# bennyguo/instant-nsr-pl

Measured on NVIDIA H100. Metric: rays/sec fwd+bwd (NeRF-Synthetic lego shape), higher is better.
Workload: dtype f16

## Files before the change

instant-nsr-pl_b200/csrc/nerf_fused_bwd.cu:

```cuda
#include <stdlib.h>
#include "nerf_fused.cuh"
#include "wgmma.cuh"

namespace {

constexpr int kWarps = 4;
constexpr int kThreads = kWarps * 32;
constexpr int kRows = kWarps * 16;
constexpr int kCtasPerSm = 2;

constexpr int T_X0 = 0;
constexpr int T_H1 = T_X0 + kRows * NF_LD32;
constexpr int T_CI = T_H1 + kRows * NSR_LD64;
constexpr int T_G1 = T_CI + kRows * NF_LD32;
constexpr int T_G2 = T_G1 + kRows * NSR_LD64;
constexpr int T_DC3 = T_G2 + kRows * NSR_LD64;
constexpr int T_DG2 = T_DC3 + kRows * 24;
constexpr int T_DG1 = T_DG2 + kRows * NSR_LD64;
constexpr int T_DO = T_DG1 + kRows * NSR_LD64;
constexpr int T_DH1 = T_DO + kRows * 24;
constexpr int T_X0B = T_DH1 + kRows * NSR_LD64;
constexpr int T_TOTAL = T_X0B + kRows * NF_LD32;
constexpr int S_XYZ = 0, S_DS = S_XYZ + kRows * 6, S_DRGB = S_DS + kRows, S_ROWF = S_DRGB + kRows * 3;
constexpr size_t kSmemBytes = (size_t)(NF_W_TOTAL + T_TOTAL) * sizeof(__half) + 2 * S_ROWF * sizeof(float);

__device__ __forceinline__ void cp_async16(void* smem_dst, const void* gsrc) {
  asm volatile("cp.async.cg.shared.global [%0], [%1], 16;" ::"r"((uint32_t)__cvta_generic_to_shared(smem_dst)), "l"(gsrc) : "memory");
}
__device__ __forceinline__ void cp_async_commit() { asm volatile("cp.async.commit_group;" ::: "memory"); }
__device__ __forceinline__ void cp_async_wait_all() { asm volatile("cp.async.wait_group 0;" ::: "memory"); }

constexpr int kSlots = 40 / kWarps;

struct WgradTile {
  int dy_off, ldy, x_off, ldx, m0, n0;
  int net, base, in_dim;
};

__device__ __forceinline__ WgradTile wgrad_tile(int t) {
  WgradTile w;
  if (t < 8) {
    w = {T_DH1, NSR_LD64, T_X0, NF_LD32, (t / 2) * 16, (t % 2) * 16, 0, 0, 32};
  } else if (t < 12) {
    w = {T_DO, 24, T_H1, NSR_LD64, 0, (t - 8) * 16, 0, 64 * 32, 64};
  } else if (t < 20) {
    const int u = t - 12;
    w = {T_DG1, NSR_LD64, T_CI, NF_LD32, (u / 2) * 16, (u % 2) * 16, 1, 0, 32};
  } else if (t < 36) {
    const int u = t - 20;
    w = {T_DG2, NSR_LD64, T_G1, NSR_LD64, (u / 4) * 16, (u % 4) * 16, 1, 64 * 32, 64};
  } else {
    w = {T_DC3, 24, T_G2, NSR_LD64, 0, (t - 36) * 16, 1, 64 * 32 + 64 * 64, 64};
  }
  return w;
}

__device__ __forceinline__ void relu_mask_pack(const float (&acc)[1][8][4], const uint32_t (&post)[1][4][4], uint32_t (&out)[1][4][4]) {
#pragma unroll
  for (int k = 0; k < 4; ++k)
#pragma unroll
    for (int j = 0; j < 4; ++j) {
      const __half2 hv = *reinterpret_cast<const __half2*>(&post[0][k][j]);
      const int nt = 2 * k + (j >> 1), i0 = (j & 1) * 2;
      const float d0 = __low2float(hv) > 0.f ? acc[0][nt][i0] : 0.f;
      const float d1 = __high2float(hv) > 0.f ? acc[0][nt][i0 + 1] : 0.f;
      out[0][k][j] = nsr_pack_h2(d0, d1);
    }
}

template <bool PACKED>
__global__ void __launch_bounds__(kThreads, kCtasPerSm) nerf_bwd_kernel(const __grid_constant__ nsr_nerf_t P, const float* __restrict__ rays,
                                                               const int32_t* __restrict__ ray_indices, const float* __restrict__ t_starts,
                                                               const float* __restrict__ t_ends, const __half* __restrict__ enc_save,
                                                               const __half* __restrict__ dparams, const __half* __restrict__ cparams,
                                                               const float* __restrict__ d_sraw, const float* __restrict__ d_rgb,
                                                               float* __restrict__ grad_dparams, float* __restrict__ grad_cparams,
                                                               float loss_scale, const float* __restrict__ amax_ptr, int64_t n_cap, const int64_t* __restrict__ n_dev,
                                                               const int64_t* __restrict__ row_pos, const float* __restrict__ xyzdir) {
  const int64_t n = n_dev ? min(*n_dev, n_cap) : n_cap;
  extern __shared__ __align__(16) __half smem[];
  __half* T = smem + NF_W_TOTAL;
  float* rowf = reinterpret_cast<float*>(smem + NF_W_TOTAL + T_TOTAL);
  const int warp = threadIdx.x >> 5, lane = threadIdx.x & 31, g = lane >> 2, c = lane & 3;
  const int r0 = warp * 16;
  if (loss_scale <= 0.f) {
    const float amax = fmaxf(__ldg(amax_ptr), 1e-30f);
    loss_scale = exp2f(fminf(fmaxf(floorf(log2f(256.f / amax)), -24.f), 60.f));
  }
  const float inv_scale = 1.f / loss_scale;
  nf_stage_weights(smem, dparams, cparams, true);
  float* grad_table = grad_dparams + NF_DENSITY_PARAMS;

  float wacc[kSlots][2][4];
#pragma unroll
  for (int s = 0; s < kSlots; ++s)
#pragma unroll
    for (int j = 0; j < 2; ++j)
#pragma unroll
      for (int i = 0; i < 4; ++i) wacc[s][j][i] = 0.f;

  const int64_t n_tiles = (n + kRows - 1) / kRows;
  auto fetch_tile = [&](int64_t tile, int buf) {
    const int64_t row0 = tile * kRows;
    __half* xb = T + (buf ? T_X0B : T_X0);
    float* rf = rowf + buf * S_ROWF;
    for (int v = threadIdx.x; v < kRows * 4; v += kThreads)
      cp_async16(xb + (v >> 2) * NF_LD32 + (v & 3) * 8, enc_save + (row0 + (v >> 2)) * 32 + (v & 3) * 8);
    for (int v = threadIdx.x; v < kRows * 6 / 4; v += kThreads) cp_async16(rf + S_XYZ + v * 4, xyzdir + row0 * 6 + v * 4);
    if (threadIdx.x < kRows / 4) cp_async16(rf + S_DS + threadIdx.x * 4, d_sraw + row0 + threadIdx.x * 4);
    if (threadIdx.x >= 64 && threadIdx.x < 64 + kRows * 3 / 4)
      cp_async16(rf + S_DRGB + (threadIdx.x - 64) * 4, d_rgb + row0 * 3 + (threadIdx.x - 64) * 4);
    cp_async_commit();
  };
  int buf = 0;
  if (PACKED && (int64_t)blockIdx.x < n_tiles) fetch_tile(blockIdx.x, 0);
  for (int64_t tile = blockIdx.x; tile < n_tiles; tile += gridDim.x, buf ^= 1) {
    const int64_t row0 = tile * kRows;
    if (PACKED) cp_async_wait_all();
    __syncthreads();
    const __half* X0 = T + ((PACKED && buf) ? T_X0B : T_X0);
    const int x0_off = (PACKED && buf) ? T_X0B : T_X0;
    const float* rf = rowf + buf * S_ROWF;
    if (PACKED) {
      if (tile + gridDim.x < n_tiles) fetch_tile(tile + gridDim.x, buf ^ 1);
      if (row0 + kRows > n) {
        for (int v = threadIdx.x; v < kRows * 4; v += kThreads)
          if (row0 + (v >> 2) >= n) *reinterpret_cast<uint4*>(T + x0_off + (v >> 2) * NF_LD32 + (v & 3) * 8) = make_uint4(0, 0, 0, 0);
        float* rw = rowf + buf * S_ROWF;
        for (int v = threadIdx.x; v < S_ROWF; v += kThreads) {
          const int r = v < S_DS ? v / 6 : (v < S_DRGB ? v - S_DS : (v - S_DRGB) / 3);
          if (row0 + r >= n) rw[v] = 0.f;
        }
        __syncthreads();
      }
    }
    const int64_t ia = row0 + r0 + g, ib = ia + 8;
    const int64_t pa = (!PACKED && row_pos && ia < n) ? row_pos[ia] : ia, pb = (!PACKED && row_pos && ib < n) ? row_pos[ib] : ib;
    if (!PACKED) {
      for (int v = lane; v < 64; v += 32) {
        const int r = v >> 2, q = v & 3;
        const int64_t i = row0 + r0 + r;
        uint4 val = make_uint4(0, 0, 0, 0);
        if (i < n) val = __ldg(reinterpret_cast<const uint4*>(enc_save + (row_pos ? row_pos[i] : i) * 32) + q);
        *reinterpret_cast<uint4*>(T + T_X0 + (r0 + r) * NF_LD32 + q * 8) = val;
      }
    }
    if (lane < 16) {
      const int64_t i = row0 + r0 + lane;
      uint4 s0 = make_uint4(0, 0, 0, 0), s1 = s0;
      if (i < n) {
        float s[16];
        if (PACKED) {
          const float* rr = rf + S_XYZ + (r0 + lane) * 6;
          nsr_sh4(rr[3], rr[4], rr[5], s);
        } else {
          const float* rr = rays + (size_t)ray_indices[i] * 6;
          nsr_sh4(__ldg(rr + 3), __ldg(rr + 4), __ldg(rr + 5), s);
        }
        s0 = make_uint4(nsr_pack_h2(s[0], s[1]), nsr_pack_h2(s[2], s[3]), nsr_pack_h2(s[4], s[5]), nsr_pack_h2(s[6], s[7]));
        s1 = make_uint4(nsr_pack_h2(s[8], s[9]), nsr_pack_h2(s[10], s[11]), nsr_pack_h2(s[12], s[13]), nsr_pack_h2(s[14], s[15]));
      }
      uint4* sp = reinterpret_cast<uint4*>(T + T_CI + (r0 + lane) * NF_LD32 + 16);
      sp[0] = s0;
      sp[1] = s1;
    }
    __syncwarp();

    uint32_t a_h1[1][4][4], a_o[1][1][4], a_g1[1][4][4], a_g2[1][4][4];
    float acc[1][8][4], acc16[1][2][4];
    {
      uint32_t a_in[1][2][4];
      nsr_load_afrag<1, 2>(a_in, X0, NF_LD32, r0);
      nsr_zero_acc(acc);
      nsr_gemm_w<1, 2, 8>(acc, a_in, smem + NF_OFF_DW1, NF_LD32);
      nsr_acc_to_afrag<1, 8>(acc, a_h1, NSR_ACT_RELU);
      nsr_store_afrag<1, 4>(a_h1, T + T_H1, NSR_LD64, r0);
      nsr_zero_acc(acc16);
      nsr_gemm_w<1, 4, 2>(acc16, a_h1, smem + NF_OFF_DW2, NSR_LD64);
      nsr_acc_to_afrag<1, 2>(acc16, a_o, NSR_ACT_NONE);
      nsr_store_afrag<1, 1>(a_o, T + T_CI, NF_LD32, r0, 0);
    }
    {
      uint32_t a_c[1][2][4], a_sh[1][1][4];
      nsr_load_afrag<1, 1>(a_sh, T + T_CI + 16, NF_LD32, r0);
#pragma unroll
      for (int j = 0; j < 4; ++j) {
        a_c[0][0][j] = a_o[0][0][j];
        a_c[0][1][j] = a_sh[0][0][j];
      }
      nsr_zero_acc(acc);
      nsr_gemm_w<1, 2, 8>(acc, a_c, smem + NF_OFF_CW1, NF_LD32);
      nsr_acc_to_afrag<1, 8>(acc, a_g1, NSR_ACT_RELU);
      nsr_store_afrag<1, 4>(a_g1, T + T_G1, NSR_LD64, r0);
      nsr_zero_acc(acc);
      nsr_gemm_w<1, 4, 8>(acc, a_g1, smem + NF_OFF_CW2, NSR_LD64);
      nsr_acc_to_afrag<1, 8>(acc, a_g2, NSR_ACT_RELU);
      nsr_store_afrag<1, 4>(a_g2, T + T_G2, NSR_LD64, r0);
      nsr_zero_acc(acc16);
      nsr_gemm_w<1, 4, 2>(acc16, a_g2, smem + NF_OFF_CW3, NSR_LD64);
    }
    uint32_t a_dc3[1][1][4];
    {
      float dp[4] = {0.f, 0.f, 0.f, 0.f};
      if (c < 2) {
#pragma unroll
        for (int hh = 0; hh < 2; ++hh) {
          const int64_t i = hh ? ib : ia, pi = hh ? pb : pa;
          if (i < n) {
#pragma unroll
            for (int e = 0; e < 2; ++e) {
              const int col = c * 2 + e;
              if (col < 3) {
                const float raw = __half2float(__float2half_rn(acc16[0][0][hh * 2 + e]));
                const float s = 1.f / (1.f + expf(-raw));
                const float dr = PACKED ? rf[S_DRGB + (r0 + g + hh * 8) * 3 + col] : d_rgb[pi * 3 + col];
                dp[hh * 2 + e] = dr * s * (1.f - s) * loss_scale;
              }
            }
          }
        }
      }
      a_dc3[0][0][0] = nsr_pack_h2(dp[0], dp[1]);
      a_dc3[0][0][1] = nsr_pack_h2(dp[2], dp[3]);
      a_dc3[0][0][2] = 0u;
      a_dc3[0][0][3] = 0u;
      nsr_store_afrag<1, 1>(a_dc3, T + T_DC3, 24, r0);
    }
    uint32_t a_d[1][4][4];
    nsr_zero_acc(acc);
    nsr_gemm_wt<1, 1, 8>(acc, a_dc3, smem + NF_OFF_CW3, NSR_LD64);
    relu_mask_pack(acc, a_g2, a_d);
    nsr_store_afrag<1, 4>(a_d, T + T_DG2, NSR_LD64, r0);
    nsr_zero_acc(acc);
    nsr_gemm_wt<1, 4, 8>(acc, a_d, smem + NF_OFF_CW2, NSR_LD64);
    relu_mask_pack(acc, a_g1, a_d);
    nsr_store_afrag<1, 4>(a_d, T + T_DG1, NSR_LD64, r0);
    nsr_zero_acc(acc16);
    nsr_gemm_wt<1, 4, 2>(acc16, a_d, smem + NF_OFF_CW1, NF_LD32);
    if (c == 0) {
      if (ia < n) acc16[0][0][0] += (PACKED ? rf[S_DS + r0 + g] : d_sraw[pa]) * loss_scale;
      if (ib < n) acc16[0][0][2] += (PACKED ? rf[S_DS + r0 + g + 8] : d_sraw[pb]) * loss_scale;
    }
    uint32_t a_do[1][1][4];
    nsr_acc_to_afrag<1, 2>(acc16, a_do, NSR_ACT_NONE);
    nsr_store_afrag<1, 1>(a_do, T + T_DO, 24, r0);
    nsr_zero_acc(acc);
    nsr_gemm_wt<1, 1, 8>(acc, a_do, smem + NF_OFF_DW2, NSR_LD64);
    relu_mask_pack(acc, a_h1, a_d);
    nsr_store_afrag<1, 4>(a_d, T + T_DH1, NSR_LD64, r0);
    float accE[1][4][4];
    nsr_zero_acc(accE);
    nsr_gemm_wt<1, 4, 4>(accE, a_d, smem + NF_OFF_DW1, NF_LD32);

#pragma unroll
    for (int hh = 0; hh < 2; ++hh) {
      const int64_t i = hh ? ib : ia;
      const bool ok = i < n;
      float x = 0.f, y = 0.f, z = 0.f, dx, dy, dz;
      if (ok) {
        if (PACKED) {
          const float* rr = rf + S_XYZ + (r0 + g + hh * 8) * 6;
          x = rr[0];
          y = rr[1];
          z = rr[2];
        } else {
          nf_sample_position(P, rays, ray_indices[i], t_starts[i], t_ends[i], x, y, z, dx, dy, dz);
        }
      }
#pragma unroll
      for (int nt = 0; nt < 4; ++nt) {
        const float d0 = ok ? accE[0][nt][hh * 2] * inv_scale : 0.f, d1 = ok ? accE[0][nt][hh * 2 + 1] * inv_scale : 0.f;
        const LevelInfo li = nsr_level(P.grid, nt * 4 + c);
        uint32_t cx, cy, cz, idx[8];
        float fx, fy, fz;
        nsr_pos_fract(x, li.scale, cx, fx);
        nsr_pos_fract(y, li.scale, cy, fy);
        nsr_pos_fract(z, li.scale, cz, fz);
        if (nt < 2) {
          const uint32_t key = ok ? (cx + li.res * (cy + li.res * cz)) : (0xFFFFFFF0u + g);
          const uint32_t key_prev = __shfl_up_sync(0xffffffffu, key, 4);
          const bool head = (g == 0) || (key_prev != key);
          const int next_head = __shfl_down_sync(0xffffffffu, (int)head, 4);
          const bool tail = (g == 7) || next_head;
          float v[16];
#pragma unroll
          for (int cc = 0; cc < 8; ++cc) {
            const float w = nsr_corner_weight(cc, fx, fy, fz);
            v[2 * cc] = w * d0;
            v[2 * cc + 1] = w * d1;
          }
          bool flag = head;
#pragma unroll
          for (int o = 1; o < 8; o <<= 1) {
            const int f_up = __shfl_up_sync(0xffffffffu, (int)flag, 4 * o);
            const bool take = (g >= o) && !flag;
#pragma unroll
            for (int e = 0; e < 16; ++e) {
              const float u = __shfl_up_sync(0xffffffffu, v[e], 4 * o);
              if (take) v[e] += u;
            }
            if (take) flag = f_up;
          }
          if (ok && tail) {
            nsr_corner_indices(li, cx, cy, cz, idx);
#pragma unroll
            for (int cc = 0; cc < 8; ++cc)
              if (v[2 * cc] != 0.f || v[2 * cc + 1] != 0.f) nsr_red_add_f32x2(grad_table + 2 * (size_t)idx[cc], v[2 * cc], v[2 * cc + 1]);
          }
        } else if (ok && (d0 != 0.f || d1 != 0.f)) {
          nsr_corner_indices(li, cx, cy, cz, idx);
#pragma unroll
          for (int cc = 0; cc < 8; ++cc) {
            const float w = nsr_corner_weight(cc, fx, fy, fz);
            nsr_red_add_f32x2(grad_table + 2 * (size_t)idx[cc], w * d0, w * d1);
          }
        }
      }
    }
    __syncthreads();
#pragma unroll
    for (int s = 0; s < kSlots; ++s) {
      const WgradTile w = wgrad_tile(warp + s * kWarps);
      const int xo = (w.x_off == T_X0) ? x0_off : w.x_off;
      nsr_wgrad_tile(wacc[s][0], wacc[s][1], T + w.dy_off, w.ldy, w.m0, T + xo, w.ldx, w.n0, kRows);
    }
  }
#pragma unroll
  for (int s = 0; s < kSlots; ++s) {
    const WgradTile w = wgrad_tile(warp + s * kWarps);
    float* dst = (w.net == 0 ? grad_dparams : grad_cparams) + w.base;
#pragma unroll
    for (int j = 0; j < 2; ++j)
#pragma unroll
      for (int i = 0; i < 4; ++i) {
        const int o = w.m0 + g + ((i >> 1) << 3), ii = w.n0 + j * 8 + c * 2 + (i & 1);
        atomicAdd(dst + (size_t)o * w.in_dim + ii, wacc[s][j][i] * inv_scale);
      }
  }
}

constexpr int kNetThreads = 384;
constexpr int SL_X0 = 0;
constexpr int SL_CI = SL_X0 + kRows * 32 * 2;
constexpr int SL_H1 = SL_CI + kRows * 32 * 2;
constexpr int SL_G1 = SL_H1 + kRows * 64 * 2;
constexpr int SL_G2 = SL_G1 + kRows * 64 * 2;
constexpr int SL_DC3 = SL_G2 + kRows * 64 * 2;
constexpr int SL_DO = SL_DC3 + kRows * 16 * 2;
constexpr int SL_DG2 = SL_DO + kRows * 16 * 2;
constexpr int SL_DG1 = SL_DG2 + kRows * 64 * 2;
constexpr int SL_DH1 = SL_DG1 + kRows * 64 * 2;
constexpr int kSlotBytes = SL_DH1 + kRows * 64 * 2;
constexpr int kNetSlots = 3;
constexpr int N_SLOTS = NF_W_TOTAL * 2;
constexpr int N_STAGE = N_SLOTS + kNetSlots * kSlotBytes;
constexpr int kStageBytes = kRows * NF_LD32 * 2 + S_ROWF * 4;
constexpr int N_BARS = N_STAGE + 2 * kStageBytes;
constexpr size_t kNetSmemBytes = N_BARS + 2 * kNetSlots * 8;
static_assert(N_SLOTS % 128 == 0 && kSlotBytes % 128 == 0 && kStageBytes % 16 == 0 && N_BARS % 8 == 0, "alignment");
static_assert(kNetSmemBytes <= 227 * 1024, "shared memory");

template <int KT>
__device__ __forceinline__ void canon_load_afrag(uint32_t (&a)[1][KT][4], const uint8_t* tile, int K, int row0, int col0 = 0) {
  const int lane = threadIdx.x & 31, mi = lane >> 3, r = lane & 7;
#pragma unroll
  for (int k = 0; k < KT; ++k) nsr_ldmatrix_x4(a[0][k], tile + nsr_canon_off(row0 + (mi & 1) * 8 + r, col0 + k * 16 + (mi >> 1) * 8, K));
}
template <int KT>
__device__ __forceinline__ void canon_store_afrag(const uint32_t (&a)[1][KT][4], uint8_t* tile, int K, int row0, int col0 = 0) {
  const int lane = threadIdx.x & 31, g = lane >> 2, c = lane & 3;
#pragma unroll
  for (int k = 0; k < KT; ++k) {
    const int col = col0 + k * 16 + c * 2;
    *reinterpret_cast<uint32_t*>(tile + nsr_canon_off(row0 + g, col, K)) = a[0][k][0];
    *reinterpret_cast<uint32_t*>(tile + nsr_canon_off(row0 + g + 8, col, K)) = a[0][k][1];
    *reinterpret_cast<uint32_t*>(tile + nsr_canon_off(row0 + g, col + 8, K)) = a[0][k][2];
    *reinterpret_cast<uint32_t*>(tile + nsr_canon_off(row0 + g + 8, col + 8, K)) = a[0][k][3];
  }
}
__device__ __forceinline__ void group_bar(int grp) { asm volatile("bar.sync %0, 128;" ::"r"(1 + grp) : "memory"); }

template <int R>
__device__ __forceinline__ void net_flush(const float (&w)[R], float* dst, int stride_m, int stride_n, float inv_scale) {
  const int lane = threadIdx.x & 31, m0 = 16 * ((threadIdx.x >> 5) & 3) + (lane >> 2), c0 = 2 * (lane & 3);
#pragma unroll
  for (int r = 0; r < R; ++r) {
    const int j = r >> 2, h = (r >> 1) & 1, e = r & 1;
    atomicAdd(dst + (size_t)(m0 + 8 * h) * stride_m + (size_t)(8 * j + c0 + e) * stride_n, w[r] * inv_scale);
  }
}

__global__ void __launch_bounds__(kNetThreads, 1) nerf_bwd_net_kernel(const __half* __restrict__ enc_save, const __half* __restrict__ dparams,
                                                                      const __half* __restrict__ cparams, const float* __restrict__ d_sraw,
                                                                      const float* __restrict__ d_rgb, float* __restrict__ grad_dparams,
                                                                      float* __restrict__ grad_cparams, float loss_scale,
                                                                      const float* __restrict__ amax_ptr, int64_t n_cap,
                                                                      const int64_t* __restrict__ n_dev, const float* __restrict__ xyzdir,
                                                                      uint32_t* __restrict__ denc_out) {
  const int64_t n = n_dev ? min(*n_dev, n_cap) : n_cap;
  extern __shared__ __align__(128) uint8_t smem_net[];
  __half* W = reinterpret_cast<__half*>(smem_net);
  const int warp = threadIdx.x >> 5, lane = threadIdx.x & 31;
  if (loss_scale <= 0.f) {
    const float amax = fmaxf(__ldg(amax_ptr), 1e-30f);
    loss_scale = exp2f(fminf(fmaxf(floorf(log2f(256.f / amax)), -24.f), 60.f));
  }
  const float inv_scale = 1.f / loss_scale;
  const uint32_t sbase = nsr_smem_u32(smem_net);
  auto full_bar = [&](int s) { return sbase + N_BARS + 8u * (uint32_t)s; };
  auto empty_bar = [&](int s) { return sbase + N_BARS + 8u * (uint32_t)(kNetSlots + s); };
  if (threadIdx.x == 0) {
    for (int s = 0; s < kNetSlots; ++s) {
      mbar_init(full_bar(s), 128);
      mbar_init(empty_bar(s), 128);
    }
    asm volatile("fence.mbarrier_init.release.cluster;" ::: "memory");
  }
  nf_stage_weights(W, dparams, cparams, true);
  __syncthreads();
  const int64_t n_tiles = (n + kRows - 1) / kRows;
  const int64_t my_tiles = n_tiles > (int64_t)blockIdx.x ? (n_tiles - 1 - blockIdx.x) / gridDim.x + 1 : 0;

  if (warp < 8) {
    const int grp = warp >> 2, gtid = threadIdx.x & 127, g = lane >> 2, c = lane & 3;
    const int r0 = (warp & 3) * 16;
    __half* sx = reinterpret_cast<__half*>(smem_net + N_STAGE + grp * kStageBytes);
    float* rf = reinterpret_cast<float*>(smem_net + N_STAGE + grp * kStageBytes + kRows * NF_LD32 * 2);
    auto fetch_tile = [&](int64_t it) {
      const int64_t row0 = ((int64_t)blockIdx.x + it * gridDim.x) * kRows;
      for (int v = gtid; v < kRows * 4; v += 128) cp_async16(sx + (v >> 2) * NF_LD32 + (v & 3) * 8, enc_save + (row0 + (v >> 2)) * 32 + (v & 3) * 8);
      if (gtid < kRows * 6 / 4) cp_async16(rf + S_XYZ + gtid * 4, xyzdir + row0 * 6 + gtid * 4);
      if (gtid < kRows / 4) cp_async16(rf + S_DS + gtid * 4, d_sraw + row0 + gtid * 4);
      if (gtid >= 64 && gtid < 64 + kRows * 3 / 4) cp_async16(rf + S_DRGB + (gtid - 64) * 4, d_rgb + row0 * 3 + (gtid - 64) * 4);
      cp_async_commit();
    };
    if (grp < my_tiles) fetch_tile(grp);
    for (int64_t it = grp; it < my_tiles; it += 2) {
      const int s = (int)(it % kNetSlots);
      const int64_t row0 = ((int64_t)blockIdx.x + it * gridDim.x) * kRows;
      cp_async_wait_all();
      group_bar(grp);
      if (row0 + kRows > n) {
        for (int v = gtid; v < kRows * 4; v += 128)
          if (row0 + (v >> 2) >= n) *reinterpret_cast<uint4*>(sx + (v >> 2) * NF_LD32 + (v & 3) * 8) = make_uint4(0, 0, 0, 0);
        for (int v = gtid; v < S_ROWF; v += 128) {
          const int r = v < S_DS ? v / 6 : (v < S_DRGB ? v - S_DS : (v - S_DRGB) / 3);
          if (row0 + r >= n) rf[v] = 0.f;
        }
        group_bar(grp);
      }
      if (it >= kNetSlots) mbar_wait(empty_bar(s), (uint32_t)((it / kNetSlots - 1) & 1), nullptr, 0);
      uint8_t* slot = smem_net + N_SLOTS + s * kSlotBytes;
      const int64_t ia = row0 + r0 + g, ib = ia + 8;
      uint32_t a_in[1][2][4];
      nsr_load_afrag<1, 2>(a_in, sx, NF_LD32, r0);
      canon_store_afrag<2>(a_in, slot + SL_X0, 32, r0);
      if (lane < 16) {
        uint4 s0 = make_uint4(0, 0, 0, 0), s1 = s0;
        if (row0 + r0 + lane < n) {
          float sh[16];
          const float* rr = rf + S_XYZ + (r0 + lane) * 6;
          nsr_sh4(rr[3], rr[4], rr[5], sh);
          s0 = make_uint4(nsr_pack_h2(sh[0], sh[1]), nsr_pack_h2(sh[2], sh[3]), nsr_pack_h2(sh[4], sh[5]), nsr_pack_h2(sh[6], sh[7]));
          s1 = make_uint4(nsr_pack_h2(sh[8], sh[9]), nsr_pack_h2(sh[10], sh[11]), nsr_pack_h2(sh[12], sh[13]), nsr_pack_h2(sh[14], sh[15]));
        }
        *reinterpret_cast<uint4*>(slot + SL_CI + nsr_canon_off(r0 + lane, 16, 32)) = s0;
        *reinterpret_cast<uint4*>(slot + SL_CI + nsr_canon_off(r0 + lane, 24, 32)) = s1;
      }
      float drgb[2][2], dsr[2];
#pragma unroll
      for (int hh = 0; hh < 2; ++hh) {
#pragma unroll
        for (int e = 0; e < 2; ++e) drgb[hh][e] = (c * 2 + e < 3) ? rf[S_DRGB + (r0 + g + hh * 8) * 3 + c * 2 + e] : 0.f;
        dsr[hh] = rf[S_DS + r0 + g + hh * 8];
      }
      group_bar(grp);
      if (it + 2 < my_tiles) fetch_tile(it + 2);

      uint32_t a_h1[1][4][4], a_o[1][1][4], a_g1[1][4][4], a_g2[1][4][4];
      float acc[1][8][4], acc16[1][2][4];
      nsr_zero_acc(acc);
      nsr_gemm_w<1, 2, 8>(acc, a_in, W + NF_OFF_DW1, NF_LD32);
      nsr_acc_to_afrag<1, 8>(acc, a_h1, NSR_ACT_RELU);
      canon_store_afrag<4>(a_h1, slot + SL_H1, 64, r0);
      nsr_zero_acc(acc16);
      nsr_gemm_w<1, 4, 2>(acc16, a_h1, W + NF_OFF_DW2, NSR_LD64);
      nsr_acc_to_afrag<1, 2>(acc16, a_o, NSR_ACT_NONE);
      canon_store_afrag<1>(a_o, slot + SL_CI, 32, r0);
      __syncwarp();
      {
        uint32_t a_c[1][2][4], a_sh[1][1][4];
        canon_load_afrag<1>(a_sh, slot + SL_CI, 32, r0, 16);
#pragma unroll
        for (int j = 0; j < 4; ++j) {
          a_c[0][0][j] = a_o[0][0][j];
          a_c[0][1][j] = a_sh[0][0][j];
        }
        nsr_zero_acc(acc);
        nsr_gemm_w<1, 2, 8>(acc, a_c, W + NF_OFF_CW1, NF_LD32);
      }
      nsr_acc_to_afrag<1, 8>(acc, a_g1, NSR_ACT_RELU);
      canon_store_afrag<4>(a_g1, slot + SL_G1, 64, r0);
      nsr_zero_acc(acc);
      nsr_gemm_w<1, 4, 8>(acc, a_g1, W + NF_OFF_CW2, NSR_LD64);
      nsr_acc_to_afrag<1, 8>(acc, a_g2, NSR_ACT_RELU);
      canon_store_afrag<4>(a_g2, slot + SL_G2, 64, r0);
      nsr_zero_acc(acc16);
      nsr_gemm_w<1, 4, 2>(acc16, a_g2, W + NF_OFF_CW3, NSR_LD64);
      uint32_t a_dc3[1][1][4];
      {
        float dp[4] = {0.f, 0.f, 0.f, 0.f};
        if (c < 2) {
#pragma unroll
          for (int hh = 0; hh < 2; ++hh) {
            if ((hh ? ib : ia) < n) {
#pragma unroll
              for (int e = 0; e < 2; ++e) {
                if (c * 2 + e < 3) {
                  const float raw = __half2float(__float2half_rn(acc16[0][0][hh * 2 + e]));
                  const float sg = 1.f / (1.f + expf(-raw));
                  dp[hh * 2 + e] = drgb[hh][e] * sg * (1.f - sg) * loss_scale;
                }
              }
            }
          }
        }
        a_dc3[0][0][0] = nsr_pack_h2(dp[0], dp[1]);
        a_dc3[0][0][1] = nsr_pack_h2(dp[2], dp[3]);
        a_dc3[0][0][2] = 0u;
        a_dc3[0][0][3] = 0u;
        canon_store_afrag<1>(a_dc3, slot + SL_DC3, 16, r0);
      }
      uint32_t a_d[1][4][4];
      nsr_zero_acc(acc);
      nsr_gemm_wt<1, 1, 8>(acc, a_dc3, W + NF_OFF_CW3, NSR_LD64);
      relu_mask_pack(acc, a_g2, a_d);
      canon_store_afrag<4>(a_d, slot + SL_DG2, 64, r0);
      nsr_zero_acc(acc);
      nsr_gemm_wt<1, 4, 8>(acc, a_d, W + NF_OFF_CW2, NSR_LD64);
      relu_mask_pack(acc, a_g1, a_d);
      canon_store_afrag<4>(a_d, slot + SL_DG1, 64, r0);
      nsr_zero_acc(acc16);
      nsr_gemm_wt<1, 4, 2>(acc16, a_d, W + NF_OFF_CW1, NF_LD32);
      if (c == 0) {
        if (ia < n) acc16[0][0][0] += dsr[0] * loss_scale;
        if (ib < n) acc16[0][0][2] += dsr[1] * loss_scale;
      }
      uint32_t a_do[1][1][4];
      nsr_acc_to_afrag<1, 2>(acc16, a_do, NSR_ACT_NONE);
      canon_store_afrag<1>(a_do, slot + SL_DO, 16, r0);
      nsr_zero_acc(acc);
      nsr_gemm_wt<1, 1, 8>(acc, a_do, W + NF_OFF_DW2, NSR_LD64);
      relu_mask_pack(acc, a_h1, a_d);
      canon_store_afrag<4>(a_d, slot + SL_DH1, 64, r0);
      nsr_proxy_fence();
      mbar_arrive(full_bar(s));
      float accE[1][4][4];
      nsr_zero_acc(accE);
      nsr_gemm_wt<1, 4, 4>(accE, a_d, W + NF_OFF_DW1, NF_LD32);
#pragma unroll
      for (int hh = 0; hh < 2; ++hh) {
        const int64_t i = hh ? ib : ia;
        if (i < n) {
#pragma unroll
          for (int nt = 0; nt < 4; ++nt) denc_out[i * 16 + nt * 4 + c] = nsr_pack_h2(accE[0][nt][hh * 2], accE[0][nt][hh * 2 + 1]);
        }
      }
    }
  } else {
    float w_dw1[16], w_dw2t[8], w_cw1[16], w_cw2[32], w_cw3t[8];
#pragma unroll
    for (int i = 0; i < 32; ++i) {
      if (i < 8) w_dw2t[i] = w_cw3t[i] = 0.f;
      if (i < 16) w_dw1[i] = w_cw1[i] = 0.f;
      w_cw2[i] = 0.f;
    }
    for (int64_t it = 0; it < my_tiles; ++it) {
      const int s = (int)(it % kNetSlots);
      mbar_wait(full_bar(s), (uint32_t)((it / kNetSlots) & 1), nullptr, 0);
      const uint32_t sl = sbase + N_SLOTS + (uint32_t)s * kSlotBytes;
      nsr_wg_fence();
#pragma unroll
      for (int kk = 0; kk < 4; ++kk) {
        nsr_wgmma_n32<1, 1>(w_dw1, nsr_wg_desc_mn(sl + SL_DH1, 64, kk), nsr_wg_desc_mn(sl + SL_X0, 32, kk), 1u);
        nsr_wgmma_n16<1, 1>(w_dw2t, nsr_wg_desc_mn(sl + SL_H1, 64, kk), nsr_wg_desc_mn(sl + SL_DO, 16, kk), 1u);
        nsr_wgmma_n32<1, 1>(w_cw1, nsr_wg_desc_mn(sl + SL_DG1, 64, kk), nsr_wg_desc_mn(sl + SL_CI, 32, kk), 1u);
        nsr_wgmma_n64<1, 1>(w_cw2, nsr_wg_desc_mn(sl + SL_DG2, 64, kk), nsr_wg_desc_mn(sl + SL_G1, 64, kk), 1u);
        nsr_wgmma_n16<1, 1>(w_cw3t, nsr_wg_desc_mn(sl + SL_G2, 64, kk), nsr_wg_desc_mn(sl + SL_DC3, 16, kk), 1u);
      }
      nsr_wg_commit();
      nsr_wg_wait0();
      nsr_wg_fence_regs(w_dw1);
      nsr_wg_fence_regs(w_dw2t);
      nsr_wg_fence_regs(w_cw1);
      nsr_wg_fence_regs(w_cw2);
      nsr_wg_fence_regs(w_cw3t);
      mbar_arrive(empty_bar(s));
    }
    if (my_tiles > 0) {
      net_flush(w_dw1, grad_dparams, 32, 1, inv_scale);
      net_flush(w_dw2t, grad_dparams + 64 * 32, 1, 64, inv_scale);
      net_flush(w_cw1, grad_cparams, 32, 1, inv_scale);
      net_flush(w_cw2, grad_cparams + 64 * 32, 64, 1, inv_scale);
      net_flush(w_cw3t, grad_cparams + 64 * 32 + 64 * 64, 1, 64, inv_scale);
    }
  }
}

}

namespace {

constexpr int kMergeLevels = 8;

template <int MINB>
__global__ void __launch_bounds__(256, MINB) nerf_table_scatter_kernel(const __grid_constant__ nsr_grid_t g, const float* __restrict__ xyz, int stride,
                                                                 const __half2* __restrict__ denc, float loss_scale,
                                                                 const float* __restrict__ amax_ptr, float* __restrict__ grad_table,
                                                                 int64_t n_cap, const int64_t* __restrict__ n_dev, int l_begin, int l_end) {
  const int64_t n = n_dev ? min(*n_dev, n_cap) : n_cap;
  if (loss_scale <= 0.f) {
    const float amax = fmaxf(__ldg(amax_ptr), 1e-30f);
    loss_scale = exp2f(fminf(fmaxf(floorf(log2f(256.f / amax)), -24.f), 60.f));
  }
  const float inv_scale = 1.f / loss_scale;
  const int lane = threadIdx.x & 31;
  const int64_t n32 = (n + 31) & ~31ll;
  for (int64_t i = blockIdx.x * 256ll + threadIdx.x; i < n32; i += (int64_t)gridDim.x * 256) {
    const bool ok = i < n;
    float x = 0.f, y = 0.f, z = 0.f;
    if (ok) {
      x = xyz[i * stride];
      y = xyz[i * stride + 1];
      z = xyz[i * stride + 2];
    }
    uint2 dq = make_uint2(0u, 0u);
#pragma unroll 1
    for (int l = l_begin; l < l_end; ++l) {
      float2 d = make_float2(0.f, 0.f);
      if (ok) {
        if (l == l_begin || (l & 1) == 0) dq = __ldg(reinterpret_cast<const uint2*>(denc + i * 16 + (l & ~1)));
        const uint32_t h = (l & 1) ? dq.y : dq.x;
        d = __half22float2(*reinterpret_cast<const __half2*>(&h));
        d.x *= inv_scale;
        d.y *= inv_scale;
      }
      const LevelInfo li = nsr_level(g, l);
      uint32_t cx, cy, cz, idx[8];
      float fx, fy, fz;
      nsr_pos_fract(x, li.scale, cx, fx);
      nsr_pos_fract(y, li.scale, cy, fy);
      nsr_pos_fract(z, li.scale, cz, fz);
      float v[16];
#pragma unroll
      for (int c = 0; c < 8; ++c) {
        const float w = nsr_corner_weight(c, fx, fy, fz);
        v[2 * c] = w * d.x;
        v[2 * c + 1] = w * d.y;
      }
      bool issue = ok && (d.x != 0.f || d.y != 0.f);
      if (l < kMergeLevels) {
        const uint32_t key = ok ? (cx + li.res * (cy + li.res * cz)) : (0xFFFFFF00u + lane);
        const uint32_t prev = __shfl_up_sync(0xffffffffu, key, 1);
        const bool head = lane == 0 || prev != key;
        const uint32_t heads = __ballot_sync(0xffffffffu, head);
        const int my_head = 31 - __clz(heads & (0xffffffffu >> (31 - lane)));
        const bool tail = lane == 31 || ((heads >> (lane + 1)) & 1u);
        int maxrun = lane - my_head + 1;
#pragma unroll
        for (int o = 16; o > 0; o >>= 1) maxrun = max(maxrun, __shfl_xor_sync(0xffffffffu, maxrun, o));
#pragma unroll
        for (int o = 1; o < 32; o <<= 1) {
          if (o < maxrun) {
            const bool take = lane - o >= my_head;
#pragma unroll
            for (int e = 0; e < 16; ++e) {
              const float u = __shfl_up_sync(0xffffffffu, v[e], o);
              if (take) v[e] += u;
            }
          }
        }
        issue = ok && tail;
      }
      if (issue) {
        nsr_corner_indices(li, cx, cy, cz, idx);
#pragma unroll
        for (int c = 0; c < 8; c += 2) nsr_red_corner_pair(grad_table, idx[c], idx[c + 1], v[2 * c], v[2 * c + 1], v[2 * c + 2], v[2 * c + 3]);
      }
    }
  }
}

int field_bwd_launch(const nsr_nerf_t* f, const float* rays, const int32_t* ray_indices, const float* t_starts, const float* t_ends,
                     const void* enc_save_h, const void* dparams_h, const void* cparams_h, const float* d_sraw, const float* d_rgb,
                     float* grad_dparams, float* grad_cparams, float loss_scale, const float* amax, int64_t k, const int64_t* k_dev,
                     const int64_t* row_pos, const float* xyzdir, void* stream, const char* who) {
  NSR_REQUIRE(f != nullptr, "%s: field descriptor is NULL", who);
  NSR_REQUIRE(f->grid.n_levels == 16 && f->grid.n_features == 2 && f->feature_dim == 16 && f->density_hidden == 1 && f->color_hidden == 2,
              "%s: fused path needs L=16, F=2, feature_dim=16, hidden layers 1/2", who);
  NSR_REQUIRE(loss_scale > 0.f || amax != nullptr, "%s: loss_scale <= 0 (automatic) needs the amax pointer", who);
  if (k == 0) return 0;
  NSR_REQUIRE(xyzdir == nullptr || row_pos == nullptr, "%s: packed inputs (xyzdir) and row_pos are mutually exclusive", who);
  static thread_local bool attr_set = false;
  if (!attr_set) {
    cudaError_t e = cudaFuncSetAttribute(nerf_bwd_kernel<false>, cudaFuncAttributeMaxDynamicSharedMemorySize, (int)kSmemBytes);
    if (e == cudaSuccess) e = cudaFuncSetAttribute(nerf_bwd_kernel<true>, cudaFuncAttributeMaxDynamicSharedMemorySize, (int)kSmemBytes);
    if (e != cudaSuccess) {
      nsr_set_error("%s: cannot reserve %zu B shared memory: %s", who, kSmemBytes, cudaGetErrorString(e));
      return 2;
    }
    attr_set = true;
  }
  const int64_t tiles = (k + kRows - 1) / kRows;
  int grid = (int)min((int64_t)nsr_sm_count() * kCtasPerSm, tiles);
  if (k_dev != nullptr) grid = nsr_sm_count() * kCtasPerSm;
#define NSR_BWD_ARGS                                                                                                                        \
  *f, rays, ray_indices, t_starts, t_ends, (const __half*)enc_save_h, (const __half*)dparams_h, (const __half*)cparams_h, d_sraw, d_rgb,    \
      grad_dparams, grad_cparams, loss_scale, amax, k, k_dev, row_pos, xyzdir
  if (xyzdir != nullptr)
    nerf_bwd_kernel<true><<<grid, kThreads, kSmemBytes, (cudaStream_t)stream>>>(NSR_BWD_ARGS);
// ... 96 lines not shown
```

Baseline: 14.79 million.

## Add third compute group to net backward kernel and reload activations from smem

Restructures the warp-specialized backward net kernel so it runs three 128-thread compute groups, one per pipeline slot, instead of two, with the wgmma weight-gradient warpgroup moved to the first 128 threads. Post-activation tiles are no longer held in registers; they are reloaded from shared memory with ldmatrix before each ReLU mask, which lowers register pressure enough for the larger block. Input-tile register loads and SH encoding now happen before the wait on the empty slot, so the next prefetch can be issued earlier. In exchange the block uses more threads and more stage shared memory and issues extra shared-memory reads, and the single wgmma group now has to keep up with three producers.

```diff
diff --git a/instant-nsr-pl_b200/csrc/nerf_fused_bwd.cu b/instant-nsr-pl_b200/csrc/nerf_fused_bwd.cu
--- a/instant-nsr-pl_b200/csrc/nerf_fused_bwd.cu
+++ b/instant-nsr-pl_b200/csrc/nerf_fused_bwd.cu
@@ -55,17 +55,20 @@
   return w;
 }
 
-__device__ __forceinline__ void relu_mask_pack(const float (&acc)[1][8][4], const uint32_t (&post)[1][4][4], uint32_t (&out)[1][4][4]) {
-#pragma unroll
-  for (int k = 0; k < 4; ++k)
-#pragma unroll
-    for (int j = 0; j < 4; ++j) {
-      const __half2 hv = *reinterpret_cast<const __half2*>(&post[0][k][j]);
-      const int nt = 2 * k + (j >> 1), i0 = (j & 1) * 2;
-      const float d0 = __low2float(hv) > 0.f ? acc[0][nt][i0] : 0.f;
-      const float d1 = __high2float(hv) > 0.f ? acc[0][nt][i0 + 1] : 0.f;
-      out[0][k][j] = nsr_pack_h2(d0, d1);
-    }
+template <int MT>
+__device__ __forceinline__ void relu_mask_pack(const float (&acc)[MT][8][4], const uint32_t (&post)[MT][4][4], uint32_t (&out)[MT][4][4]) {
+#pragma unroll
+  for (int m = 0; m < MT; ++m)
+#pragma unroll
+    for (int k = 0; k < 4; ++k)
+#pragma unroll
+      for (int j = 0; j < 4; ++j) {
+        const __half2 hv = *reinterpret_cast<const __half2*>(&post[m][k][j]);
+        const int nt = 2 * k + (j >> 1), i0 = (j & 1) * 2;
+        const float d0 = __low2float(hv) > 0.f ? acc[m][nt][i0] : 0.f;
+        const float d1 = __high2float(hv) > 0.f ? acc[m][nt][i0 + 1] : 0.f;
+        out[m][k][j] = nsr_pack_h2(d0, d1);
+      }
 }
 
 template <bool PACKED>
@@ -339,7 +342,11 @@
   }
 }
 
-constexpr int kNetThreads = 384;
+constexpr int kNetSlots = 3;
+constexpr int kNetGroups = kNetSlots;
+constexpr int kNetWgThreads = 128;
+constexpr int kNetGroupThreads = 128;
+constexpr int kNetThreads = kNetWgThreads + kNetGroups * kNetGroupThreads;
 constexpr int SL_X0 = 0;
 constexpr int SL_CI = SL_X0 + kRows * 32 * 2;
 constexpr int SL_H1 = SL_CI + kRows * 32 * 2;
@@ -351,34 +358,38 @@
 constexpr int SL_DG1 = SL_DG2 + kRows * 64 * 2;
 constexpr int SL_DH1 = SL_DG1 + kRows * 64 * 2;
 constexpr int kSlotBytes = SL_DH1 + kRows * 64 * 2;
-constexpr int kNetSlots = 3;
 constexpr int N_SLOTS = NF_W_TOTAL * 2;
 constexpr int N_STAGE = N_SLOTS + kNetSlots * kSlotBytes;
 constexpr int kStageBytes = kRows * NF_LD32 * 2 + S_ROWF * 4;
-constexpr int N_BARS = N_STAGE + 2 * kStageBytes;
+constexpr int N_BARS = N_STAGE + kNetGroups * kStageBytes;
 constexpr size_t kNetSmemBytes = N_BARS + 2 * kNetSlots * 8;
 static_assert(N_SLOTS % 128 == 0 && kSlotBytes % 128 == 0 && kStageBytes % 16 == 0 && N_BARS % 8 == 0, "alignment");
 static_assert(kNetSmemBytes <= 227 * 1024, "shared memory");
 
-template <int KT>
-__device__ __forceinline__ void canon_load_afrag(uint32_t (&a)[1][KT][4], const uint8_t* tile, int K, int row0, int col0 = 0) {
+template <int MT, int KT>
+__device__ __forceinline__ void canon_load_afrag(uint32_t (&a)[MT][KT][4], const uint8_t* tile, int K, int row0, int col0 = 0) {
   const int lane = threadIdx.x & 31, mi = lane >> 3, r = lane & 7;
 #pragma unroll
-  for (int k = 0; k < KT; ++k) nsr_ldmatrix_x4(a[0][k], tile + nsr_canon_off(row0 + (mi & 1) * 8 + r, col0 + k * 16 + (mi >> 1) * 8, K));
-}
-template <int KT>
-__device__ __forceinline__ void canon_store_afrag(const uint32_t (&a)[1][KT][4], uint8_t* tile, int K, int row0, int col0 = 0) {
+  for (int m = 0; m < MT; ++m)
+#pragma unroll
+    for (int k = 0; k < KT; ++k)
+      nsr_ldmatrix_x4(a[m][k], tile + nsr_canon_off(row0 + m * 16 + (mi & 1) * 8 + r, col0 + k * 16 + (mi >> 1) * 8, K));
+}
+template <int MT, int KT>
+__device__ __forceinline__ void canon_store_afrag(const uint32_t (&a)[MT][KT][4], uint8_t* tile, int K, int row0, int col0 = 0) {
   const int lane = threadIdx.x & 31, g = lane >> 2, c = lane & 3;
 #pragma unroll
-  for (int k = 0; k < KT; ++k) {
-    const int col = col0 + k * 16 + c * 2;
-    *reinterpret_cast<uint32_t*>(tile + nsr_canon_off(row0 + g, col, K)) = a[0][k][0];
-    *reinterpret_cast<uint32_t*>(tile + nsr_canon_off(row0 + g + 8, col, K)) = a[0][k][1];
-    *reinterpret_cast<uint32_t*>(tile + nsr_canon_off(row0 + g, col + 8, K)) = a[0][k][2];
-    *reinterpret_cast<uint32_t*>(tile + nsr_canon_off(row0 + g + 8, col + 8, K)) = a[0][k][3];
-  }
-}
-__device__ __forceinline__ void group_bar(int grp) { asm volatile("bar.sync %0, 128;" ::"r"(1 + grp) : "memory"); }
+  for (int m = 0; m < MT; ++m)
+#pragma unroll
+    for (int k = 0; k < KT; ++k) {
+      const int row = row0 + m * 16 + g, col = col0 + k * 16 + c * 2;
+      *reinterpret_cast<uint32_t*>(tile + nsr_canon_off(row, col, K)) = a[m][k][0];
+      *reinterpret_cast<uint32_t*>(tile + nsr_canon_off(row + 8, col, K)) = a[m][k][1];
+      *reinterpret_cast<uint32_t*>(tile + nsr_canon_off(row, col + 8, K)) = a[m][k][2];
+      *reinterpret_cast<uint32_t*>(tile + nsr_canon_off(row + 8, col + 8, K)) = a[m][k][3];
+    }
+}
+__device__ __forceinline__ void group_bar(int grp) { asm volatile("bar.sync %0, %1;" ::"r"(1 + grp), "n"(kNetGroupThreads) : "memory"); }
 
 template <int R>
 __device__ __forceinline__ void net_flush(const float (&w)[R], float* dst, int stride_m, int stride_n, float inv_scale) {
@@ -411,8 +422,8 @@
   auto empty_bar = [&](int s) { return sbase + N_BARS + 8u * (uint32_t)(kNetSlots + s); };
   if (threadIdx.x == 0) {
     for (int s = 0; s < kNetSlots; ++s) {
-      mbar_init(full_bar(s), 128);
-      mbar_init(empty_bar(s), 128);
+      mbar_init(full_bar(s), kNetGroupThreads);
+      mbar_init(empty_bar(s), kNetWgThreads);
     }
     asm volatile("fence.mbarrier_init.release.cluster;" ::: "memory");
   }
@@ -421,151 +432,168 @@
   const int64_t n_tiles = (n + kRows - 1) / kRows;
   const int64_t my_tiles = n_tiles > (int64_t)blockIdx.x ? (n_tiles - 1 - blockIdx.x) / gridDim.x + 1 : 0;
 
-  if (warp < 8) {
-    const int grp = warp >> 2, gtid = threadIdx.x & 127, g = lane >> 2, c = lane & 3;
-    const int r0 = (warp & 3) * 16;
+  if (threadIdx.x >= kNetWgThreads) {
+    const int grp = threadIdx.x / kNetGroupThreads - 1, gtid = threadIdx.x % kNetGroupThreads, g = lane >> 2, c = lane & 3;
     __half* sx = reinterpret_cast<__half*>(smem_net + N_STAGE + grp * kStageBytes);
     float* rf = reinterpret_cast<float*>(smem_net + N_STAGE + grp * kStageBytes + kRows * NF_LD32 * 2);
     auto fetch_tile = [&](int64_t it) {
       const int64_t row0 = ((int64_t)blockIdx.x + it * gridDim.x) * kRows;
-      for (int v = gtid; v < kRows * 4; v += 128) cp_async16(sx + (v >> 2) * NF_LD32 + (v & 3) * 8, enc_save + (row0 + (v >> 2)) * 32 + (v & 3) * 8);
-      if (gtid < kRows * 6 / 4) cp_async16(rf + S_XYZ + gtid * 4, xyzdir + row0 * 6 + gtid * 4);
+      for (int v = gtid; v < kRows * 4; v += kNetGroupThreads)
+        cp_async16(sx + (v >> 2) * NF_LD32 + (v & 3) * 8, enc_save + (row0 + (v >> 2)) * 32 + (v & 3) * 8);
+      for (int v = gtid; v < kRows * 6 / 4; v += kNetGroupThreads) cp_async16(rf + S_XYZ + v * 4, xyzdir + row0 * 6 + v * 4);
       if (gtid < kRows / 4) cp_async16(rf + S_DS + gtid * 4, d_sraw + row0 + gtid * 4);
-      if (gtid >= 64 && gtid < 64 + kRows * 3 / 4) cp_async16(rf + S_DRGB + (gtid - 64) * 4, d_rgb + row0 * 3 + (gtid - 64) * 4);
+      else if (gtid < kRows / 4 + kRows * 3 / 4) cp_async16(rf + S_DRGB + (gtid - kRows / 4) * 4, d_rgb + row0 * 3 + (gtid - kRows / 4) * 4);
       cp_async_commit();
     };
+    constexpr int MT = 1;
+    const int r0 = (gtid >> 5) * 16 * MT;
     if (grp < my_tiles) fetch_tile(grp);
-    for (int64_t it = grp; it < my_tiles; it += 2) {
+    for (int64_t it = grp; it < my_tiles; it += kNetGroups) {
       const int s = (int)(it % kNetSlots);
       const int64_t row0 = ((int64_t)blockIdx.x + it * gridDim.x) * kRows;
       cp_async_wait_all();
       group_bar(grp);
       if (row0 + kRows > n) {
-        for (int v = gtid; v < kRows * 4; v += 128)
+        for (int v = gtid; v < kRows * 4; v += kNetGroupThreads)
           if (row0 + (v >> 2) >= n) *reinterpret_cast<uint4*>(sx + (v >> 2) * NF_LD32 + (v & 3) * 8) = make_uint4(0, 0, 0, 0);
-        for (int v = gtid; v < S_ROWF; v += 128) {
+        for (int v = gtid; v < S_ROWF; v += kNetGroupThreads) {
           const int r = v < S_DS ? v / 6 : (v < S_DRGB ? v - S_DS : (v - S_DRGB) / 3);
           if (row0 + r >= n) rf[v] = 0.f;
         }
         group_bar(grp);
       }
+      uint32_t a_in[MT][2][4];
+      nsr_load_afrag<MT, 2>(a_in, sx, NF_LD32, r0);
+      uint4 sh0 = make_uint4(0, 0, 0, 0), sh1 = sh0;
+      if (lane < 16 * MT && row0 + r0 + lane < n) {
+        float sh[16];
+        const float* rr = rf + S_XYZ + (r0 + lane) * 6;
+        nsr_sh4(rr[3], rr[4], rr[5], sh);
+        sh0 = make_uint4(nsr_pack_h2(sh[0], sh[1]), nsr_pack_h2(sh[2], sh[3]), nsr_pack_h2(sh[4], sh[5]), nsr_pack_h2(sh[6], sh[7]));
+        sh1 = make_uint4(nsr_pack_h2(sh[8], sh[9]), nsr_pack_h2(sh[10], sh[11]), nsr_pack_h2(sh[12], sh[13]), nsr_pack_h2(sh[14], sh[15]));
+      }
+      float drgb[MT][2][2], dsr[MT][2];
+#pragma unroll
+      for (int m = 0; m < MT; ++m)
+#pragma unroll
+        for (int hh = 0; hh < 2; ++hh) {
+          const int r = r0 + m * 16 + g + hh * 8;
+#pragma unroll
+          for (int e = 0; e < 2; ++e) drgb[m][hh][e] = (c * 2 + e < 3) ? rf[S_DRGB + r * 3 + c * 2 + e] : 0.f;
+          dsr[m][hh] = rf[S_DS + r];
+        }
+      group_bar(grp);
+      if (it + kNetGroups < my_tiles) fetch_tile(it + kNetGroups);
       if (it >= kNetSlots) mbar_wait(empty_bar(s), (uint32_t)((it / kNetSlots - 1) & 1), nullptr, 0);
       uint8_t* slot = smem_net + N_SLOTS + s * kSlotBytes;
-      const int64_t ia = row0 + r0 + g, ib = ia + 8;
-      uint32_t a_in[1][2][4];
-      nsr_load_afrag<1, 2>(a_in, sx, NF_LD32, r0);
-      canon_store_afrag<2>(a_in, slot + SL_X0, 32, r0);
-      if (lane < 16) {
-        uint4 s0 = make_uint4(0, 0, 0, 0), s1 = s0;
-        if (row0 + r0 + lane < n) {
-          float sh[16];
-          const float* rr = rf + S_XYZ + (r0 + lane) * 6;
-          nsr_sh4(rr[3], rr[4], rr[5], sh);
-          s0 = make_uint4(nsr_pack_h2(sh[0], sh[1]), nsr_pack_h2(sh[2], sh[3]), nsr_pack_h2(sh[4], sh[5]), nsr_pack_h2(sh[6], sh[7]));
-          s1 = make_uint4(nsr_pack_h2(sh[8], sh[9]), nsr_pack_h2(sh[10], sh[11]), nsr_pack_h2(sh[12], sh[13]), nsr_pack_h2(sh[14], sh[15]));
-        }
-        *reinterpret_cast<uint4*>(slot + SL_CI + nsr_canon_off(r0 + lane, 16, 32)) = s0;
-        *reinterpret_cast<uint4*>(slot + SL_CI + nsr_canon_off(r0 + lane, 24, 32)) = s1;
-      }
-      float drgb[2][2], dsr[2];
-#pragma unroll
-      for (int hh = 0; hh < 2; ++hh) {
-#pragma unroll
-        for (int e = 0; e < 2; ++e) drgb[hh][e] = (c * 2 + e < 3) ? rf[S_DRGB + (r0 + g + hh * 8) * 3 + c * 2 + e] : 0.f;
-        dsr[hh] = rf[S_DS + r0 + g + hh * 8];
-      }
-      group_bar(grp);
-      if (it + 2 < my_tiles) fetch_tile(it + 2);
-
-      uint32_t a_h1[1][4][4], a_o[1][1][4], a_g1[1][4][4], a_g2[1][4][4];
-      float acc[1][8][4], acc16[1][2][4];
+      canon_store_afrag<MT, 2>(a_in, slot + SL_X0, 32, r0);
+      if (lane < 16 * MT) {
+        *reinterpret_cast<uint4*>(slot + SL_CI + nsr_canon_off(r0 + lane, 16, 32)) = sh0;
+        *reinterpret_cast<uint4*>(slot + SL_CI + nsr_canon_off(r0 + lane, 24, 32)) = sh1;
+      }
+
+      uint32_t a_h[MT][4][4];
+      float acc[MT][8][4], acc16[MT][2][4];
       nsr_zero_acc(acc);
-      nsr_gemm_w<1, 2, 8>(acc, a_in, W + NF_OFF_DW1, NF_LD32);
-      nsr_acc_to_afrag<1, 8>(acc, a_h1, NSR_ACT_RELU);
-      canon_store_afrag<4>(a_h1, slot + SL_H1, 64, r0);
+      nsr_gemm_w<MT, 2, 8>(acc, a_in, W + NF_OFF_DW1, NF_LD32);
+      nsr_acc_to_afrag<MT, 8>(acc, a_h, NSR_ACT_RELU);
+      canon_store_afrag<MT, 4>(a_h, slot + SL_H1, 64, r0);
       nsr_zero_acc(acc16);
-      nsr_gemm_w<1, 4, 2>(acc16, a_h1, W + NF_OFF_DW2, NSR_LD64);
-      nsr_acc_to_afrag<1, 2>(acc16, a_o, NSR_ACT_NONE);
-      canon_store_afrag<1>(a_o, slot + SL_CI, 32, r0);
-      __syncwarp();
+      nsr_gemm_w<MT, 4, 2>(acc16, a_h, W + NF_OFF_DW2, NSR_LD64);
       {
-        uint32_t a_c[1][2][4], a_sh[1][1][4];
-        canon_load_afrag<1>(a_sh, slot + SL_CI, 32, r0, 16);
-#pragma unroll
-        for (int j = 0; j < 4; ++j) {
-          a_c[0][0][j] = a_o[0][0][j];
-          a_c[0][1][j] = a_sh[0][0][j];
-        }
+        uint32_t a_c[MT][2][4], a_o[MT][1][4], a_sh[MT][1][4];
+        nsr_acc_to_afrag<MT, 2>(acc16, a_o, NSR_ACT_NONE);
+        canon_store_afrag<MT, 1>(a_o, slot + SL_CI, 32, r0);
+        __syncwarp();
+        canon_load_afrag<MT, 1>(a_sh, slot + SL_CI, 32, r0, 16);
+#pragma unroll
+        for (int m = 0; m < MT; ++m)
+#pragma unroll
+          for (int j = 0; j < 4; ++j) {
+            a_c[m][0][j] = a_o[m][0][j];
+            a_c[m][1][j] = a_sh[m][0][j];
+          }
         nsr_zero_acc(acc);
-        nsr_gemm_w<1, 2, 8>(acc, a_c, W + NF_OFF_CW1, NF_LD32);
-      }
-      nsr_acc_to_afrag<1, 8>(acc, a_g1, NSR_ACT_RELU);
-      canon_store_afrag<4>(a_g1, slot + SL_G1, 64, r0);
+        nsr_gemm_w<MT, 2, 8>(acc, a_c, W + NF_OFF_CW1, NF_LD32);
+      }
+      nsr_acc_to_afrag<MT, 8>(acc, a_h, NSR_ACT_RELU);
+      canon_store_afrag<MT, 4>(a_h, slot + SL_G1, 64, r0);
       nsr_zero_acc(acc);
-      nsr_gemm_w<1, 4, 8>(acc, a_g1, W + NF_OFF_CW2, NSR_LD64);
-      nsr_acc_to_afrag<1, 8>(acc, a_g2, NSR_ACT_RELU);
-      canon_store_afrag<4>(a_g2, slot + SL_G2, 64, r0);
+      nsr_gemm_w<MT, 4, 8>(acc, a_h, W + NF_OFF_CW2, NSR_LD64);
+      nsr_acc_to_afrag<MT, 8>(acc, a_h, NSR_ACT_RELU);
+      canon_store_afrag<MT, 4>(a_h, slot + SL_G2, 64, r0);
       nsr_zero_acc(acc16);
-      nsr_gemm_w<1, 4, 2>(acc16, a_g2, W + NF_OFF_CW3, NSR_LD64);
-      uint32_t a_dc3[1][1][4];
-      {
+      nsr_gemm_w<MT, 4, 2>(acc16, a_h, W + NF_OFF_CW3, NSR_LD64);
+      uint32_t a_dc3[MT][1][4];
+#pragma unroll
+      for (int m = 0; m < MT; ++m) {
         float dp[4] = {0.f, 0.f, 0.f, 0.f};
         if (c < 2) {
 #pragma unroll
           for (int hh = 0; hh < 2; ++hh) {
-            if ((hh ? ib : ia) < n) {
+            if (row0 + r0 + m * 16 + g + hh * 8 < n) {
 #pragma unroll
               for (int e = 0; e < 2; ++e) {
                 if (c * 2 + e < 3) {
-                  const float raw = __half2float(__float2half_rn(acc16[0][0][hh * 2 + e]));
+                  const float raw = __half2float(__float2half_rn(acc16[m][0][hh * 2 + e]));
                   const float sg = 1.f / (1.f + expf(-raw));
-                  dp[hh * 2 + e] = drgb[hh][e] * sg * (1.f - sg) * loss_scale;
+                  dp[hh * 2 + e] = drgb[m][hh][e] * sg * (1.f - sg) * loss_scale;
                 }
               }
             }
           }
         }
-        a_dc3[0][0][0] = nsr_pack_h2(dp[0], dp[1]);
-        a_dc3[0][0][1] = nsr_pack_h2(dp[2], dp[3]);
-        a_dc3[0][0][2] = 0u;
-        a_dc3[0][0][3] = 0u;
-        canon_store_afrag<1>(a_dc3, slot + SL_DC3, 16, r0);
-      }
-      uint32_t a_d[1][4][4];
+        a_dc3[m][0][0] = nsr_pack_h2(dp[0], dp[1]);
+        a_dc3[m][0][1] = nsr_pack_h2(dp[2], dp[3]);
+        a_dc3[m][0][2] = 0u;
+        a_dc3[m][0][3] = 0u;
+      }
+      canon_store_afrag<MT, 1>(a_dc3, slot + SL_DC3, 16, r0);
+      __syncwarp();
+      uint32_t a_d[MT][4][4];
       nsr_zero_acc(acc);
-      nsr_gemm_wt<1, 1, 8>(acc, a_dc3, W + NF_OFF_CW3, NSR_LD64);
-      relu_mask_pack(acc, a_g2, a_d);
-      canon_store_afrag<4>(a_d, slot + SL_DG2, 64, r0);
+      nsr_gemm_wt<MT, 1, 8>(acc, a_dc3, W + NF_OFF_CW3, NSR_LD64);
+      canon_load_afrag<MT, 4>(a_h, slot + SL_G2, 64, r0);
+      relu_mask_pack(acc, a_h, a_d);
+      canon_store_afrag<MT, 4>(a_d, slot + SL_DG2, 64, r0);
       nsr_zero_acc(acc);
-      nsr_gemm_wt<1, 4, 8>(acc, a_d, W + NF_OFF_CW2, NSR_LD64);
-      relu_mask_pack(acc, a_g1, a_d);
-      canon_store_afrag<4>(a_d, slot + SL_DG1, 64, r0);
+      nsr_gemm_wt<MT, 4, 8>(acc, a_d, W + NF_OFF_CW2, NSR_LD64);
+      canon_load_afrag<MT, 4>(a_h, slot + SL_G1, 64, r0);
+      relu_mask_pack(acc, a_h, a_d);
+      canon_store_afrag<MT, 4>(a_d, slot + SL_DG1, 64, r0);
       nsr_zero_acc(acc16);
-      nsr_gemm_wt<1, 4, 2>(acc16, a_d, W + NF_OFF_CW1, NF_LD32);
+      nsr_gemm_wt<MT, 4, 2>(acc16, a_d, W + NF_OFF_CW1, NF_LD32);
       if (c == 0) {
-        if (ia < n) acc16[0][0][0] += dsr[0] * loss_scale;
-        if (ib < n) acc16[0][0][2] += dsr[1] * loss_scale;
-      }
-      uint32_t a_do[1][1][4];
-      nsr_acc_to_afrag<1, 2>(acc16, a_do, NSR_ACT_NONE);
-      canon_store_afrag<1>(a_do, slot + SL_DO, 16, r0);
+#pragma unroll
+        for (int m = 0; m < MT; ++m) {
+          const int64_t ia = row0 + r0 + m * 16 + g;
+          if (ia < n) acc16[m][0][0] += dsr[m][0] * loss_scale;
+          if (ia + 8 < n) acc16[m][0][2] += dsr[m][1] * loss_scale;
+        }
+      }
+      uint32_t a_do[MT][1][4];
+      nsr_acc_to_afrag<MT, 2>(acc16, a_do, NSR_ACT_NONE);
+      canon_store_afrag<MT, 1>(a_do, slot + SL_DO, 16, r0);
       nsr_zero_acc(acc);
-      nsr_gemm_wt<1, 1, 8>(acc, a_do, W + NF_OFF_DW2, NSR_LD64);
-      relu_mask_pack(acc, a_h1, a_d);
-      canon_store_afrag<4>(a_d, slot + SL_DH1, 64, r0);
+      nsr_gemm_wt<MT, 1, 8>(acc, a_do, W + NF_OFF_DW2, NSR_LD64);
+      canon_load_afrag<MT, 4>(a_h, slot + SL_H1, 64, r0);
+      relu_mask_pack(acc, a_h, a_d);
+      canon_store_afrag<MT, 4>(a_d, slot + SL_DH1, 64, r0);
       nsr_proxy_fence();
       mbar_arrive(full_bar(s));
-      float accE[1][4][4];
+      float accE[MT][4][4];
       nsr_zero_acc(accE);
-      nsr_gemm_wt<1, 4, 4>(accE, a_d, W + NF_OFF_DW1, NF_LD32);
-#pragma unroll
-      for (int hh = 0; hh < 2; ++hh) {
-        const int64_t i = hh ? ib : ia;
-        if (i < n) {
-#pragma unroll
-          for (int nt = 0; nt < 4; ++nt) denc_out[i * 16 + nt * 4 + c] = nsr_pack_h2(accE[0][nt][hh * 2], accE[0][nt][hh * 2 + 1]);
-        }
-      }
+      nsr_gemm_wt<MT, 4, 4>(accE, a_d, W + NF_OFF_DW1, NF_LD32);
+#pragma unroll
+      for (int m = 0; m < MT; ++m)
+#pragma unroll
+        for (int hh = 0; hh < 2; ++hh) {
+          const int64_t i = row0 + r0 + m * 16 + g + hh * 8;
+          if (i < n) {
+#pragma unroll
+            for (int nt = 0; nt < 4; ++nt) denc_out[i * 16 + nt * 4 + c] = nsr_pack_h2(accE[m][nt][hh * 2], accE[m][nt][hh * 2 + 1]);
+          }
+        }
     }
   } else {
     float w_dw1[16], w_dw2t[8], w_cw1[16], w_cw2[32], w_cw3t[8];
```

Result: no change. 14.93 million (median of 6 runs) (+1.0%).
